# GenomicBreeding/GenomicBreedingModels.jl

Hardware: AMD Instinct MI355X
Metric: GRM+GBLUP genotype-cells/s (n x p) (higher is better)
Workload: dtype f64

## Files before the change

### genomicbreedingmodels.jl_amd/csrc/chol.hip

```cpp
#include <cstdlib>
#include <string>

#include "chol_device.h"

namespace gbm {

constexpr int NB = kCholNB;
constexpr int MAXRHS = 63;

int launch_chol_update(double* G, int64_t ldg, int64_t k0, int64_t nb, int64_t gdim, double* Ld, double* Dinv,
                       int32_t* info, int64_t next_k0, int rank, int nranks, hipStream_t s, int64_t col_lo = 0,
                       int64_t col_hi = INT64_MAX, int64_t row_lo = 0, int64_t row_hi = INT64_MAX);
int launch_chol_row_update(double* G, int64_t ldg, int64_t k0, int kch, int64_t gdim, double* Ld, double* Dinv,
                           int32_t* info, hipStream_t s, ColKeep keep = ColKeep{});
int64_t chol_small_lim();
void chol_refresh_tuning();
int64_t chol_flow_flag_bytes(int64_t gdim);
bool chol_flow_enabled(int64_t npad);
int launch_chol_flow(double* G, int64_t ldg, int64_t gdim, double* Ld, double* Dinv, void* flag_block, int32_t* info,
                     hipStream_t s);

__global__ void __launch_bounds__(256) prepare_v_kernel(double* __restrict__ G, int64_t ld, int64_t n,
                                                        int64_t npad, int64_t gdim, double inv_q,
                                                        const int64_t* __restrict__ q_dev, double lambda,
                                                        const double* __restrict__ Y, int64_t ldy, int64_t nrhs,
                                                        int32_t* __restrict__ info, ColKeep keep) {
  const int64_t i = blockIdx.x;
  if (i == 0 && threadIdx.x == 0) *info = 0;
  if (q_dev) inv_q = 1.0 / (double)(*q_dev);
  double* row = G + i * ld;
  const int64_t jbeg = (i / NB) * NB;
  for (int64_t j = jbeg + threadIdx.x; j < gdim; j += 256) {
    if (keep.nranks > 1 && !col_kept(keep, j)) continue;
    double v = 0.0;
    if (i < npad) {
      if (j < i) v = 0.0;
      else if (j < npad) v = (i < n && j < n) ? row[j] * inv_q + (i == j ? lambda : 0.0) : (i == j ? 1.0 : 0.0);
      else if (i < n) {
        const int64_t t = j - npad;
        v = t == 0 ? 1.0 : (t <= nrhs ? Y[(t - 1) * ldy + i] : 0.0);
      }
    }
    row[j] = v;
  }
}

// ... 664 lines not shown
    const char* e = ::gbm::knob(name);
    return e ? (int64_t)atoll(e) : dflt;
  };
  const int64_t g4 = lim("GBM_CHOL_G4_LIM", 8192), g8 = lim("GBM_CHOL_G8_LIM", 8192),
                g16 = lim("GBM_CHOL_G16_LIM", 16384);
  const int64_t k0 = kb * NB;
  if (g16 >= 0 && kb + 16 < nb && gdim - (k0 + 16 * NB) > g16) return 16;
  if (g8 >= 0 && kb + 8 < nb && gdim - (k0 + 8 * NB) > g8) return 8;
  if (g4 >= 0 && kb + 4 < nb && gdim - (k0 + 4 * NB) > g4) return 4;
  if (kb + 2 < nb && gdim - (k0 + 2 * NB) > chol_small_lim()) return 2;
  return 1;
}

int solve_prepare(double* G, int64_t ldg, int64_t n, double inv_q, const int64_t* q_dev, double lambda,
                  const double* Y, int64_t ldy, int64_t nrhs, int32_t* info, void* workspace, hipStream_t s,
                  bool factor_first = true, ColKeep keep = ColKeep{}) {
  const int64_t npad = npad_of(n), gdim = gdim_of(n);
  const SolveWs w = solve_ws(workspace, npad);
  chol_refresh_tuning();
  prepare_v_kernel<<<(unsigned)gdim, 256, 0, s>>>(G, ldg, n, npad, gdim, inv_q, q_dev, lambda, Y, ldy, nrhs, info,
                                                  keep);
  GBM_LAUNCH_CHECK();
  if (!factor_first) return GBM_OK;
  factor_diag_kernel<<<1, 256, 0, s>>>(G, ldg, 0, w.Ld, w.Dinv, info);
  GBM_LAUNCH_CHECK();
  return GBM_OK;
}

static bool group_kernel_enabled() {
  const char* e = ::gbm::knob("GBM_CHOL_GROUP_KERNEL");
  return !e || atoi(e) != 0;
}

int solve_group_panels(double* G, int64_t ldg, int64_t n, int64_t kb, ColKeep keep, int32_t* info, void* workspace,
                       hipStream_t s, int64_t* g_out) {
  const int64_t npad = npad_of(n), gdim = gdim_of(n), nb = npad / NB;
// ... 120 lines not shown
    GBM_TRY(solve_prepare(G, ldg, n, inv_q, q_dev, lambda, Y, ldy, nrhs, info, workspace, s, false));
    const SolveWs w = solve_ws(workspace, npad);
    GBM_TRY(launch_chol_flow(G, ldg, gdim_of(n), w.Ld, w.Dinv, w.flow, info, s));
    return solve_finish(G, ldg, n, Y, ldy, nrhs, lambda, A_out, gebv, lda, mu, info, workspace, s);
  }
  GBM_TRY(solve_prepare(G, ldg, n, inv_q, q_dev, lambda, Y, ldy, nrhs, info, workspace, s));
  const int64_t nb = npad / NB;
  for (int64_t kb = 0; kb < nb;) {
    int64_t g = 1;
    GBM_TRY(solve_group(G, ldg, n, kb, info, workspace, s, &g));
    kb += g;
  }
  return solve_finish(G, ldg, n, Y, ldy, nrhs, lambda, A_out, gebv, lda, mu, info, workspace, s);
}

extern "C" int gbm_dev_chol_prepare(double* G, int64_t ldg, int64_t n, double inv_q, const int64_t* q_dev,
                                    double lambda, const double* Y, int64_t ldy, int64_t nrhs, int32_t* info,
                                    void* workspace, int64_t ws_bytes, void* stream) {
  if (!Y || ldy < n || nrhs < 1 || nrhs > MAXRHS || !(lambda > 0.0) || !(q_dev || inv_q > 0.0))
    return fail(GBM_E_ARG, "gbm_dev_chol_prepare: bad arguments");
  GBM_TRY(check_solve_args(G, ldg, n, info, workspace, ws_bytes, "gbm_dev_chol_prepare"));
  return solve_prepare(G, ldg, n, inv_q, q_dev, lambda, Y, ldy, nrhs, info, workspace, (hipStream_t)stream);
}

extern "C" int gbm_dev_chol_prepare_cols(double* G, int64_t ldg, int64_t n, double inv_q, const int64_t* q_dev,
                                         double lambda, const double* Y, int64_t ldy, int64_t nrhs, int rank,
                                         int nranks, int32_t* info, void* workspace, int64_t ws_bytes, void* stream) {
  if (!Y || ldy < n || nrhs < 1 || nrhs > MAXRHS || !(lambda > 0.0) || !(q_dev || inv_q > 0.0) || nranks < 1 ||
      rank < 0 || rank >= nranks)
    return fail(GBM_E_ARG, "gbm_dev_chol_prepare_cols: bad arguments");
// ... 191 lines not shown
```

### genomicbreedingmodels.jl_amd/csrc/chol_device.h

```cpp
#pragma once
#include "gbm_internal.h"

namespace gbm {

typedef double d4 __attribute__((ext_vector_type(4)));

constexpr int CNB = 64;
constexpr int PS = CNB + 16;

struct ColKeep {
  int32_t rank = 0, nranks = 1;
  int64_t keep_hi = 0, rhs0 = INT64_MAX;
};
__device__ __forceinline__ bool col_kept(const ColKeep& k, int64_t col) {
  return k.nranks == 1 || col < k.keep_hi || col >= k.rhs0 || (col / 128) % k.nranks == k.rank;
}

__device__ __forceinline__ double rsqrt_nr(double a) {
  double y = __builtin_amdgcn_rsq(a);
  const double h = 0.5 * a * y;
  return y * fma(-h, y, 1.5);
}
__device__ __forceinline__ double rcp_nr(double a) {
  double y = __builtin_amdgcn_rcp(a);
  const double e = fma(-a, y, 1.0);
  return fma(y, e, y);
}
__device__ __forceinline__ double readlane_d(double x, int lane) {
  union {
    double d;
// ... 188 lines not shown
```

### genomicbreedingmodels.jl_amd/csrc/chol_flow.hip

```cpp
#include <atomic>
#include <cstdlib>
#include <map>
#include <mutex>
#include <type_traits>
#include <vector>

#include "chol_device.h"

namespace gbm {

namespace {

typedef double dbl2 __attribute__((ext_vector_type(2)));
typedef unsigned int u4 __attribute__((ext_vector_type(4)));
typedef unsigned int u2 __attribute__((ext_vector_type(2)));
constexpr int FT = 64;
constexpr int32_t kPairBit = 0x8000;
constexpr int kTraceRec = 32;
constexpr int kSc1 = 16;

__device__ __forceinline__ __amdgpu_buffer_rsrc_t rsrc(const void* p, int64_t bytes) {
  return __builtin_amdgcn_make_buffer_rsrc(const_cast<void*>(p), (short)0, (int)bytes, 0x00020000);
}
__device__ __forceinline__ dbl2 ld2(__amdgpu_buffer_rsrc_t r, uint32_t voff, uint32_t soff) {
  return __builtin_bit_cast(dbl2, __builtin_amdgcn_raw_buffer_load_b128(r, (int)voff, (int)soff, kSc1));
}
__device__ __forceinline__ double ld1(__amdgpu_buffer_rsrc_t r, uint32_t voff) {
  return __builtin_bit_cast(double, __builtin_amdgcn_raw_buffer_load_b64(r, (int)voff, 0, kSc1));
}
__device__ __forceinline__ void st2(__amdgpu_buffer_rsrc_t r, uint32_t voff, dbl2 v) {
  __builtin_amdgcn_raw_buffer_store_b128(__builtin_bit_cast(u4, v), r, (int)voff, 0, kSc1);
}
__device__ __forceinline__ void st1(__amdgpu_buffer_rsrc_t r, uint32_t voff, double v) {
  __builtin_amdgcn_raw_buffer_store_b64(__builtin_bit_cast(u2, v), r, (int)voff, 0, kSc1);
}

#ifndef GBM_FLOW_POST_EVERY
#define GBM_FLOW_POST_EVERY 4
#endif
#ifndef GBM_FLOW_STAGES
#define GBM_FLOW_STAGES 8
#endif
#ifndef GBM_FLOW_POLL_SLEEP
#define GBM_FLOW_POLL_SLEEP 4
#endif


constexpr int32_t kPartial = 1, kAssisted = 2, kFinal = 3;
__device__ __forceinline__ bool flag_at_least(const int32_t* f, int32_t v) {
// ... 287 lines not shown
  asm volatile("s_waitcnt vmcnt(0)" ::: "memory");
  if (lane == 0) __hip_atomic_fetch_or(leaf_bits, 1 << w, __ATOMIC_RELAXED, __HIP_MEMORY_SCOPE_AGENT);
  after_own(w);
  lds_sync();
  const double dg = X[lane * PS + lane];
  const unsigned long long bm = __ballot(!(dg > 0.0) || !isfinite(dg));
  return bm ? (int)__builtin_ctzll(bm) : -1;
}


template <bool kTrace>
__global__ void __launch_bounds__(256, 1)
chol_flow_kernel(double* __restrict__ G, int64_t ld, int nbc, double* __restrict__ Ld, double* __restrict__ Dinv,
                 int32_t* __restrict__ queue, int32_t* __restrict__ flags, int32_t* __restrict__ info,
                 const int32_t* __restrict__ order, int nwork, int xn_defer, int64_t* __restrict__ trace,
                 int trace_roles) {
  __shared__ __attribute__((aligned(16))) double X[FT * PS];
  __shared__ __attribute__((aligned(16))) double X2[FT * PS];
  __shared__ __attribute__((aligned(16))) double X3[FT * PS];
  __shared__ __attribute__((aligned(16))) double Dl[4 * 256];
  __shared__ ChainSync sy;
  __shared__ int s_task;
  const int tid = threadIdx.x, lane = tid & 63, wave = tid >> 6;
  const int wr = wave >> 1, wc = wave & 1;
  const int fr = lane >> 4, fc = lane & 15;
  const int nb = nbc - 1;
  const int ntasks = nbc * (nbc + 1) / 2;
  const int64_t gbytes_rowblk = (int64_t)FT * ld * 8;
  const __amdgpu_buffer_rsrc_t rLd = rsrc(Ld, (int64_t)nb * FT * CNB * 8);
  const __amdgpu_buffer_rsrc_t rDi = rsrc(Dinv, (int64_t)nb * FT * 16 * 8);

  auto store_lower = [&](const double* Xs, int64_t i0, int64_t j0) {
    const int row = tid & 63, quarter = tid >> 6;
    double* dl = G + (j0 + row) * ld + i0 + quarter * 16;
#pragma unroll
    for (int e = 0; e < 16; e += 2) {
      dbl2 v;
      v.x = Xs[(quarter * 16 + e) * PS + row];
      v.y = Xs[(quarter * 16 + e + 1) * PS + row];
      *reinterpret_cast<dbl2*>(dl + e) = v;
    }
  };

  if (blockIdx.x == 0) {
    if (tid == 0) {
      sy.rows = sy.b12 = sy.b13 = sy.pro = sy.x2 = sy.dl = 0;
    }
    for (int e = tid; e < FT * FT / 2; e += 256) {
      const int r = e >> 5, c2 = (e & 31) * 2;
      *reinterpret_cast<dbl2*>(&X[r * PS + c2]) = *reinterpret_cast<const dbl2*>(G + (int64_t)r * ld + c2);
    }
    lds_sync();
    double* Xa = X;
    double* Xn = X3;
    for (int i = 0; i < nb; i++) {
      const int64_t i0 = (int64_t)i * FT, j0 = i0 + FT;
      const bool next_diag = i + 1 < nb;
      int64_t* const crec = kTrace && (trace_roles & 1) ? trace + (int64_t)(ntasks + i) * kTraceRec : nullptr;
      auto cstamp = [&](int e, int64_t v) {
        if (kTrace && crec && tid == 0) crec[3 + e] = v;
      };
      cstamp(0, (int64_t)__builtin_amdgcn_s_memrealtime());
      __builtin_amdgcn_s_setprio(2);
      auto fetch_tile = [&](double* dst, int64_t r0, const int32_t* f, int32_t ready, auto&& gate) {
        const __amdgpu_buffer_rsrc_t rG = rsrc(G + r0 * ld, gbytes_rowblk);
// ... 181 lines not shown
  auto worker_task = [&](auto nt, int t, int i, int j) {
    constexpr int NT = decltype(nt)::value;
    const bool diag = i == j;
    const bool nbr = j == i + 1;
    if ((diag && i < nb) || nbr || j == i + 2) __builtin_amdgcn_s_setprio(2);
    const int64_t i0 = (int64_t)i * FT, j0 = (int64_t)j * FT;
    const int kend = ((diag && i < nb) || (nbr && i >= 1)) ? i - 1 : i;
    int64_t* const wrec = kTrace && (trace_roles & 4) ? trace + (int64_t)t * kTraceRec : nullptr;
    auto wstamp = [&](int e) {
      if (kTrace && wrec && tid == 0) wrec[3 + e] = (int64_t)__builtin_amdgcn_s_memrealtime();
    };
    wstamp(0);

    d4 acc[NT][2][2];
#pragma unroll
    for (int q = 0; q < NT; q++)
#pragma unroll
      for (int m = 0; m < 2; m++)
#pragma unroll
        for (int r = 0; r < 4; r++) {
          const int64_t row = i0 + 32 * wr + 2 * (fr + 4 * r) + m;
          const dbl2 v = *reinterpret_cast<const dbl2*>(G + row * ld + j0 + q * FT + 32 * wc + 2 * fc);
          acc[q][m][0][r] = v.x;
          acc[q][m][1][r] = v.y;
        }

    constexpr int GS = NT == 1 ? 32 : 21;
    constexpr unsigned long long GM = (1ull << GS) - 1;
    int kr = 0;
    bool gave_up = false;
    auto ready_upto = [&](int k) {
      for (int64_t it = 0; k >= kr && !gave_up; it++) {
        const int g = lane / GS, kk = kr + lane % GS;
        int ok = 1;
        if (g <= NT && kk < kend) ok = flag_at_least(flags + (int64_t)kk * nbc + (g == 0 ? i : j + g - 1), kFinal) ? 1 : 0;
        const unsigned long long bm = __ballot(ok);
        unsigned long long all = bm & GM;
#pragma unroll
        for (int q = 1; q <= NT; q++) all &= (bm >> (q * GS)) & GM;
        kr += all == GM ? GS : __builtin_ctzll(~all);
// ... 300 lines not shown

}

int64_t chol_flow_flag_bytes(int64_t gdim) {
  const int64_t nbc = gdim / FT;
  return round_up(16 + nbc * nbc * 4, 16);
}

bool chol_flow_enabled(int64_t npad) {
  const char* e = ::gbm::knob("GBM_CHOL_FLOW_MAX");
  const int64_t lim = e ? (int64_t)atoll(e) : (int64_t)12288;
  return npad <= lim;
}

int launch_chol_flow(double* G, int64_t ldg, int64_t gdim, double* Ld, double* Dinv, void* flag_block, int32_t* info,
                     hipStream_t s) {
  const int64_t nbc = gdim / FT;
  const int64_t ntasks = nbc * (nbc + 1) / 2;
  if (nbc < 2 || (int64_t)FT * ldg * 8 > 0x7fffffff || nbc * nbc > 0x3fffffff || nbc > 0x7fff)
    return fail(GBM_E_ARG, "dataflow Cholesky: matrix too large for 32-bit buffer offsets");
  const int32_t* order = nullptr;
  int nwork = 0;
  GBM_TRY(flow_order_dev((int)nbc, &order, &nwork));
  GBM_HIP_TRY(hipMemsetAsync(flag_block, 0, (size_t)chol_flow_flag_bytes(gdim), s));
  if (::gbm::knob("GBM_TEST_CHOL_FLOW_ABORT")) GBM_HIP_TRY(hipMemsetAsync(info, 0xFF, sizeof(int32_t), s));
  const char* ew = ::gbm::knob("GBM_CHOL_FLOW_WGS");
  const int64_t workers = ew && atoll(ew) > 0 ? atoll(ew) : flow_cus() - 2;
  const unsigned grid = (unsigned)(2 + (nwork < workers ? nwork : (workers < 1 ? 1 : workers)));
  int32_t* q = (int32_t*)flag_block;
  const char* ex = ::gbm::knob("GBM_CHOL_FLOW_XN");
  const int xn_defer = ex && atoi(ex) == 0 ? 0 : 1;
  if (::gbm::knob("GBM_CHOL_FLOW_TRACE")) {
    const int64_t nrec = ntasks + nbc;
    if (g_trace_cap < nrec) {
      if (g_trace) (void)hipFree(g_trace);
      g_trace = nullptr;
      GBM_HIP_TRY(hipMalloc((void**)&g_trace, (size_t)nrec * kTraceRec * 8));
      g_trace_cap = nrec;
    }
    GBM_HIP_TRY(hipMemsetAsync(g_trace, 0, (size_t)nrec * kTraceRec * 8, s));
    g_trace_n = nrec;
    const int tm = atoi(::gbm::knob("GBM_CHOL_FLOW_TRACE"));
    const int roles = tm > 1 ? (tm & 7) : 7;
    if (::gbm::knob("GBM_CHOL_FLOW_TRACE_PLAIN"))
      chol_flow_kernel<false><<<grid, 256, 0, s>>>(G, ldg, (int)nbc, Ld, Dinv, q, q + 4, info, order, nwork, xn_defer, nullptr, 0);
    else
    chol_flow_kernel<true><<<grid, 256, 0, s>>>(G, ldg, (int)nbc, Ld, Dinv, q, q + 4, info, order, nwork, xn_defer, g_trace, roles);
  } else {
    chol_flow_kernel<false><<<grid, 256, 0, s>>>(G, ldg, (int)nbc, Ld, Dinv, q, q + 4, info, order, nwork, xn_defer, nullptr, 0);
  }
  GBM_LAUNCH_CHECK();
  return GBM_OK;
}

}

extern "C" int64_t gbm_debug_chol_flow_trace(int64_t* host, int64_t cap) {
  using namespace gbm;
  if (!g_trace || !host) return 0;
  const int64_t n = g_trace_n < cap ? g_trace_n : cap;
  if (hipDeviceSynchronize() != hipSuccess || hipMemcpy(host, g_trace, (size_t)n * kTraceRec * 8, hipMemcpyDeviceToHost) != hipSuccess)
    return -1;
  return n;
}
// ... 18 lines not shown
```

### genomicbreedingmodels.jl_amd/csrc/gbm_internal.h

```cpp
#pragma once
#include <hip/hip_runtime.h>
#include <stdint.h>
#include <functional>
#include <string>
#include <vector>

#include "../../include/gbm.h"

namespace gbm {

constexpr int64_t kNPadTile = 128;
constexpr int64_t kRhsRows = 64;
constexpr int kCholNB = 64;

inline int64_t round_up(int64_t x, int64_t m) { return (x + m - 1) / m * m; }
inline int64_t npad_of(int64_t n) { return round_up(n < 1 ? 1 : n, kNPadTile); }
inline int64_t gdim_of(int64_t n) { return npad_of(n) + kRhsRows; }

void set_error(const std::string& msg);
int fail(int code, const std::string& msg);
const std::string& last_error();

const char* knob(const char* name);
int64_t knob_i64(const char* name, int64_t def);
// ... 5 lines not shown
      return ::gbm::fail(GBM_E_HIP, std::string("HIP error '") + hipGetErrorString(e_) +       \
                                        "' at " __FILE__ ":" + std::to_string(__LINE__) + " (" #expr ")"); \
  } while (0)

#define GBM_LAUNCH_CHECK() GBM_HIP_TRY(hipGetLastError())

#define GBM_TRY(expr)              \
  do {                             \
    int rc_ = (expr);              \
    if (rc_ != GBM_OK) return rc_; \
  } while (0)

int launch_grm(const double* Zt, int64_t ldz, int64_t p, int64_t n, double* G, int64_t ldg,
               void* ws, int64_t ws_bytes, hipStream_t s, int accum = 0, int32_t* err_out = nullptr);
bool grm_can_accumulate(int64_t n, int64_t p);
int launch_standardize_rows(const double* Xt, int64_t ldx, int64_t p, int64_t n, double* Zt, int64_t ldz, double* mean,
                            double* sd, int32_t* keep, int64_t* q_dev, hipStream_t s, bool beside_tiles = false);
bool standardize_fits_beside_tiles(int64_t n);
int64_t grm_workspace_bytes(int64_t n, int64_t p);
int launch_grm_export(const double* G, int64_t ldg, int64_t n, double inv_q, double* out, int64_t ldo, hipStream_t s);
int launch_predict(const double* Xt, int64_t ldx, int64_t p, int64_t n, const double* b, int64_t ldb, int64_t nrhs,
                   double* partial, int64_t nchunks, double* out, int64_t ldo, hipStream_t s);
int64_t predict_chunks(int64_t n, int64_t p);
int launch_add_inplace(double* a, const double* b, int64_t n, hipStream_t s);
int launch_standardize_i8(const int8_t* D, int64_t ldd, int64_t p, int64_t n, int ploidy, double* Zt, int64_t ldz,
                          double* mean, double* sd, int32_t* keep, int64_t* q_dev, hipStream_t s);
int launch_marker_rows(const double* Zt, int64_t ldz, int64_t p, int64_t n, const double* A, int64_t lda, int64_t nrhs,
                       double inv_q, const int64_t* q_dev, const double* sd, const int32_t* keep, double* B,
                       int64_t ldb, hipStream_t s);
int launch_marker_rows_i8(const int8_t* D, int64_t ldd, int64_t p, int64_t n, int ploidy, const double* A, int64_t lda,
// ... 101 lines not shown
```

### genomicbreedingmodels.jl_amd/csrc/grm.hip

```cpp
#include <algorithm>
#include <atomic>
#include <cmath>
#include <cstdio>
#include <cstdlib>
#include <map>
#include <mutex>
#include <queue>
#include <tuple>
#include <vector>

#include "chol_device.h"

namespace gbm {

constexpr int BT = 128;
constexpr int BK = 16;
constexpr int WPS = 2;
constexpr int LROW = BT + 2;
constexpr int STAGE = 2 * BK * LROW;

__device__ __forceinline__ void tile_of(int64_t t, int64_t& ti, int64_t& tj) {
  int64_t r = (int64_t)((sqrt(8.0 * (double)t + 1.0) - 1.0) * 0.5);
  while ((r + 1) * (r + 2) / 2 <= t) r++;
  while (r * (r + 1) / 2 > t) r--;
// ... 1079 lines not shown
    return GBM_OK;
  }
  if (g.sb.carry) {
    int32_t err = 0;
    GBM_HIP_TRY(hipMemcpyAsync(&err, (const int32_t*)ws + g.ntiles, sizeof(int32_t), hipMemcpyDeviceToHost, s));
    GBM_HIP_TRY(hipStreamSynchronize(s));
    if (err < 0)
      return fail(GBM_E_HIP, "GRM in-order carry accumulation: an inter-workgroup wait timed out (G is invalid)");
    return GBM_OK;
  }
  grm_slab_reduce_kernel<<<(unsigned)g.ntiles, 256, 0, s>>>((const double*)ws, g.ntiles, g.sb.n, G, ldg, accum);
  GBM_LAUNCH_CHECK();
  return GBM_OK;
}

int launch_grm(const double* Zt, int64_t ldz, int64_t p, int64_t n, double* G, int64_t ldg, void* ws,
               int64_t ws_bytes, hipStream_t s, int accum, int32_t* err_out) {
  if (accum && !grm_can_accumulate(n, p)) return fail(GBM_E_ARG, "GRM: accumulation needs the slab split");
  int rc = launch_grm_syrk(Zt, ldz, p, n, G, ldg, ws, ws_bytes, s, accum);
  if (rc != GBM_OK) return rc;
  return launch_grm_reduce(n, p, G, ldg, ws, s, accum, err_out);
}

bool grm_can_accumulate(int64_t n, int64_t p) {
  const GrmPlan g = plan(n, p);
  return g.sb.n > 1;
}

}

// ... 113 lines not shown
```

### genomicbreedingmodels.jl_amd/gbm/_lib.py

```python
from __future__ import annotations

import ctypes
import os
import threading

import numpy as np

ABI_VERSION = 212
GBM_OK = 0
GBM_E_ARG = -1
GBM_E_NOTPD = -2
GBM_E_HIP = -3
GBM_E_RCCL = -4
GBM_E_OOM = -5
GBM_E_NODEV = -6
GBM_E_DATA = -7

LIB_PATH = os.environ.get("GBM_LIBGBM") or os.path.join(os.path.dirname(os.path.abspath(__file__)), "libgbm.so")

EXPORTS = (
    "gbm_version", "gbm_last_error", "gbm_device_count", "gbm_device_allocations", "gbm_release_device_cache",
    "gbm_gblup_fit", "gbm_gblup_fit_reml", "gbm_gblup_fit_dosage_i8", "gbm_gblup_fit_synthetic", "gbm_grm", "gbm_grm_ploidy_aware", "gbm_colstats", "gbm_predict",
    "gbm_dev_npad", "gbm_dev_gdim", "gbm_dev_grm_workspace", "gbm_dev_solve_workspace",
    "gbm_dev_synth_genotypes", "gbm_dev_expand_dosage_i8", "gbm_dev_standardize", "gbm_dev_grm",
# ... 6 lines not shown
    "gbm_dev_chol_prepare", "gbm_dev_chol_prepare_cols", "gbm_dev_chol_group_size", "gbm_dev_chol_group", "gbm_dev_chol_factor_diag",
    "gbm_dev_chol_strip_doubles", "gbm_dev_chol_strip_pack", "gbm_dev_chol_strip_unpack", "gbm_dev_chol_finish",
    "gbm_dev_grm_packed_size", "gbm_dev_grm_pack", "gbm_dev_grm_unpack",
    "gbm_debug_brr_stats", "gbm_debug_brr_shape", "gbm_debug_brr_trace", "gbm_debug_chol_flow_trace",
    "gbm_dev_synth_dosage_i8", "gbm_dev_standardize_i8", "gbm_dev_grm_accumulate", "gbm_dev_marker_effects_i8",
    "gbm_debug_oom_retries", "gbm_dev_chol_group_panels", "gbm_dev_chol_group_update", "gbm_dev_chol_strip_unpack_rows", "gbm_dev_chol_lower_copy",
    "gbm_dev_chol_area_doubles", "gbm_dev_chol_area_pack", "gbm_dev_chol_area_unpack",
    "gbm_dev_chol_group_update_cols", "gbm_dev_chol_group_update_tiles", "gbm_dev_grm_exact_workspace", "gbm_dev_grm_exact_i8",
    "gbm_gblup_fit_ex", "gbm_gblup_fit_reml_ex", "gbm_gblup_fit_dosage_i8_ex", "gbm_gblup_fit_synthetic_ex",
    "gbm_session_set_grm_mode", "gbm_session_grm_used", "gbm_debug_rccl_calls", "gbm_debug_xg_choose", "gbm_debug_chol_flow_order",
    "gbm_debug_chol_flow_order_check", "gbm_debug_chol_flow_order_size", "gbm_dev_grm_exact_status", "gbm_debug_set",
    "gbm_dev_whiten_rows", "gbm_session_gwas", "gbm_session_enet_path", "gbm_dev_standardize_grm_syrk",
    "gbm_dev_grm_symmetrize", "gbm_dev_rows_times_sym", "gbm_dev_rows_times_sym_workspace", "gbm_session_pcs",
    "gbm_debug_sym_eig", "gbm_session_pair_scan", "gbm_bayes_fit_ordinal", "gbm_debug_ordinal_math",
    "gbm_bayes_fit_multi", "gbm_debug_bayes_multi_stats", "gbm_bayes_fit_multi_rows", "gbm_debug_bayes_rows_stats",
)

GBM_GRM_DEFAULT, GBM_GRM_FP64, GBM_GRM_EXACT, GBM_GRM_AUTO, GBM_GRM_DROPIN = -1, 0, 1, 2, 3
GBM_PCS_GRM, GBM_PCS_REFERENCE = 0, 1
PCS_KINDS = {"grm": GBM_PCS_GRM, "reference": GBM_PCS_REFERENCE}
PAIR_OPS = {"mult": 0, "addnorm": 1, "raise": 2, "square": 3, "invoneplus": 4, "log10epsdivlog10eps": 5}
GRM_MODES = {None: GBM_GRM_DEFAULT, "default": GBM_GRM_DEFAULT, "fp64": GBM_GRM_FP64, "exact": GBM_GRM_EXACT,
             "auto": GBM_GRM_AUTO, "dropin": GBM_GRM_DROPIN}


def grm_mode(mode) -> int:
    if isinstance(mode, int) and mode in GRM_MODES.values():
        return mode
    try:
        return GRM_MODES[mode]
# ... 102 lines not shown
    lib.gbm_dev_grm_exact_workspace.argtypes = [I64, I64]
    lib.gbm_dev_grm_exact_i8.restype = I32
    lib.gbm_dev_grm_exact_i8.argtypes = [P, I64, I64, I64, I32, P, I64, P, P, P, P, I32, P, I64, P, P]
    lib.gbm_dev_marker_effects_i8.argtypes = [P, I64, I64, I64, I32, P, I64, I64, D, P, P, P, P, P, I64, P, P]
    for f in ("gbm_dev_grm", "gbm_dev_grm_syrk", "gbm_dev_grm_accumulate"):
        getattr(lib, f).restype = I32
        getattr(lib, f).argtypes = [P, I64, I64, I64, P, I64, P, I64, P]
    lib.gbm_dev_standardize_grm_syrk.restype = I32
    lib.gbm_dev_standardize_grm_syrk.argtypes = [P, I64, I64, I64, P, I64, P, P, P, P, P, I64, P, I64, P]
    lib.gbm_dev_grm_reduce.restype = I32
    lib.gbm_dev_grm_reduce.argtypes = [I64, I64, P, I64, P, P]
    lib.gbm_dev_grm_slices.restype = I32
    lib.gbm_dev_grm_slices.argtypes = [I64, I64]
    lib.gbm_dev_gblup_solve.restype = I32
    lib.gbm_dev_gblup_solve.argtypes = [P, I64, I64, D, P, D, P, I64, I64, P, P, I64, P, P, P, I64, P]
    lib.gbm_dev_marker_effects.restype = I32
    lib.gbm_dev_marker_effects.argtypes = [P, I64, I64, I64, P, I64, I64, D, P, P, P, P, P, I64, P, P]
    lib.gbm_dev_standardize_gather.restype = I32
    lib.gbm_dev_standardize_gather.argtypes = [P, I64, I64, P, I64, P, I64, P, P, P, P, I32, P]
    lib.gbm_dev_gblup_terms.restype = I32
    lib.gbm_dev_gblup_terms.argtypes = [P, I64, I64, I64, P, P, P]
    lib.gbm_session_create.restype = I32
    lib.gbm_session_create.argtypes = [P, I64, I64, I64, I32, ctypes.POINTER(P)]
    lib.gbm_session_create_synthetic.restype = I32
    lib.gbm_session_create_synthetic.argtypes = [U64, I64, I64, I32, ctypes.POINTER(P)]
    lib.gbm_session_create_dosage_i8.restype = I32
    lib.gbm_session_create_dosage_i8.argtypes = [P, I64, I64, I64, I32, I32, ctypes.POINTER(P)]
    lib.gbm_session_destroy.restype = None
    lib.gbm_session_destroy.argtypes = [P]
    lib.gbm_session_gblup_fit.restype = I32
# ... 149 lines not shown
```

### genomicbreedingmodels.jl_amd/gbm/sharded.py

```python
from __future__ import annotations

import ctypes

import numpy as np

from . import _lib


class TorchComm:

    def __init__(self, force: bool = False):
        import torch.distributed as dist
        self.dist = dist
        self.world_size = dist.get_world_size() if dist.is_initialized() else 1
        self.rank = dist.get_rank() if dist.is_initialized() else 0
        self.force = bool(force) and dist.is_initialized()

    def all_reduce_sum(self, t):
        if self.world_size > 1 or self.force:
            self.dist.all_reduce(t, op=self.dist.ReduceOp.SUM)

    def all_gather(self, t):
        import torch
        out = torch.empty(self.world_size * t.numel(), dtype=t.dtype, device=t.device)
# ... 197 lines not shown

def _written_by_standardize(name):
    attr = "_" + name

    def get(self):
        if self._std_pending:
            self._standardize_now()
        return getattr(self, attr)

    def put(self, value):
        setattr(self, attr, value)

    return property(get, put)


class HipShardStages:

    def __init__(self, n: int, p_local: int, nrhs: int = 1, lambda_: float = 1.0, device: int = 0):
        import torch
        self.torch = torch
        self.lib = _lib.load()
        self.n, self.p, self.nrhs, self.lam = n, p_local, nrhs, float(lambda_)
        self.dev = torch.device("cuda", device)
        lib = self.lib
        self.npad = lib.gbm_dev_npad(n)
        self.gdim = lib.gbm_dev_gdim(n)
        f64 = dict(dtype=torch.float64, device=self.dev)
        self._alloc_rows(f64)
        self.mean = torch.empty(p_local, **f64)
        self.sd = torch.empty(p_local, **f64)
# ... 55 lines not shown
    sd = _written_by_standardize("sd")
    keep = _written_by_standardize("keep")
    q = _written_by_standardize("q")

    def standardize(self):
        self._q.zero_()
        self._std_pending = True

    def _standardize_now(self):
        self._std_pending = False
        _lib.check(self.lib.gbm_dev_standardize(self._p(self.X), self.npad, self.p, self.n, self._p(self._Z), self.npad,
                                                self._p(self._mean), self._p(self._sd), self._p(self._keep),
                                                self._p(self._q), self._stream()), "standardize")

    def grm_syrk(self):
        if self._std_pending:
            self._std_pending = False
            _lib.check(self.lib.gbm_dev_standardize_grm_syrk(
                self._p(self.X), self.npad, self.p, self.n, self._p(self._Z), self.npad, self._p(self._mean),
                self._p(self._sd), self._p(self._keep), self._p(self._q), self._p(self.G), self.gdim,
                self._p(self.ws_grm), self.ws_grm_bytes, self._stream()), "standardize_grm_syrk")
            return
        _lib.check(self.lib.gbm_dev_grm_syrk(self._p(self.Z), self.npad, self.p, self.n, self._p(self.G), self.gdim,
                                             self._p(self.ws_grm), self.ws_grm_bytes, self._stream()), "grm_syrk")

    def grm_reduce(self):
        _lib.check(self.lib.gbm_dev_grm_reduce(self.n, self.p, self._p(self.G), self.gdim, self._p(self.ws_grm),
                                               self._stream()), "grm_reduce")

    def grm_rows(self):
        return self.G[: self.npad]

    def grm_pack(self):
        if getattr(self, "Gp", None) is None:
            self.Gp = self.torch.empty(self.lib.gbm_dev_grm_packed_size(self.n) + 1, dtype=self.torch.float64,
                                       device=self.dev)
        _lib.check(self.lib.gbm_dev_grm_pack(self._p(self.G), self.gdim, self.n, self._p(self.Gp), self._stream()),
                   "grm_pack")
        self.Gp[-1:].copy_(self.q)
        return self.Gp

    def grm_unpack(self):
        _lib.check(self.lib.gbm_dev_grm_unpack(self._p(self.Gp), self.n, self._p(self.G), self.gdim, self._stream()),
                   "grm_unpack")
        self.q.copy_(self.Gp[-1:])

    def solve(self):
        _lib.check(self.lib.gbm_dev_gblup_solve(self._p(self.G), self.gdim, self.n, 0.0, self._p(self.q), self.lam,
                                                self._p(self.Y), self.npad, self.nrhs, self._p(self.A),
                                                self._p(self.gebv), self.npad, self._p(self.mu), self._p(self.info),
                                                self._p(self.ws_solve), self.ws_solve_bytes, self._stream()), "solve")

    def chol_prepare(self):
        _lib.check(self.lib.gbm_dev_chol_prepare(self._p(self.G), self.gdim, self.n, 0.0, self._p(self.q), self.lam,
                                                 self._p(self.Y), self.npad, self.nrhs, self._p(self.info),
                                                 self._p(self.ws_solve), self.ws_solve_bytes, self._stream()),
                   "chol_prepare")

    def chol_prepare_cols(self, rank: int, nranks: int):
        _lib.check(self.lib.gbm_dev_chol_prepare_cols(self._p(self.G), self.gdim, self.n, 0.0, self._p(self.q),
                                                      self.lam, self._p(self.Y), self.npad, self.nrhs, rank, nranks,
                                                      self._p(self.info), self._p(self.ws_solve), self.ws_solve_bytes,
# ... 227 lines not shown
```

### include/gbm.h

```cpp
#ifndef GBM_H
#define GBM_H

#include <stdint.h>

#ifdef __cplusplus
extern "C" {
#endif

#define GBM_VERSION 212

#define GBM_OK 0
#define GBM_E_ARG (-1)
#define GBM_E_NOTPD (-2)
#define GBM_E_HIP (-3)
#define GBM_E_RCCL (-4)
#define GBM_E_OOM (-5)
#define GBM_E_NODEV (-6)
#define GBM_E_DATA (-7)

#define GBM_GRM_DEFAULT (-1)
#define GBM_GRM_FP64 0
#define GBM_GRM_EXACT 1
#define GBM_GRM_AUTO 2
#define GBM_GRM_DROPIN 3
// ... 93 lines not shown
int gbm_dev_grm_syrk(const double* Zt, int64_t ldz, int64_t p, int64_t n, double* G, int64_t ldg,
                     void* workspace, int64_t ws_bytes, void* stream);
int gbm_dev_grm_reduce(int64_t n, int64_t p, double* G, int64_t ldg, const void* workspace, void* stream);
int gbm_dev_standardize_grm_syrk(const double* Xt, int64_t ldx, int64_t p, int64_t n, double* Zt, int64_t ldz,
                                 double* mean, double* sd, int32_t* keep, int64_t* q_dev, double* G, int64_t ldg,
                                 void* workspace, int64_t ws_bytes, void* stream);
int64_t gbm_dev_grm_packed_size(int64_t n);
int gbm_dev_grm_pack(const double* G, int64_t ldg, int64_t n, double* packed, void* stream);
int gbm_dev_grm_unpack(const double* packed, int64_t n, double* G, int64_t ldg, void* stream);
int gbm_dev_grm_slices(int64_t n, int64_t p);

int gbm_dev_gblup_solve(double* G, int64_t ldg, int64_t n, double inv_q, const int64_t* q_dev, double lambda,
                        const double* Y, int64_t ldy, int64_t nrhs,
                        double* A_out, double* gebv, int64_t lda, double* mu, int32_t* info,
                        void* workspace, int64_t ws_bytes, void* stream);

int gbm_dev_chol_prepare(double* G, int64_t ldg, int64_t n, double inv_q, const int64_t* q_dev, double lambda,
                         const double* Y, int64_t ldy, int64_t nrhs, int32_t* info, void* workspace,
                         int64_t ws_bytes, void* stream);
int gbm_dev_chol_prepare_cols(double* G, int64_t ldg, int64_t n, double inv_q, const int64_t* q_dev, double lambda,
                              const double* Y, int64_t ldy, int64_t nrhs, int rank, int nranks, int32_t* info,
                              void* workspace, int64_t ws_bytes, void* stream);
int64_t gbm_dev_chol_group_size(int64_t n, int64_t kb);
int gbm_dev_chol_group(double* G, int64_t ldg, int64_t n, int64_t kb, int rank, int nranks, int32_t* info,
                       void* workspace, int64_t ws_bytes, void* stream);
int gbm_dev_chol_group_panels(double* G, int64_t ldg, int64_t n, int64_t kb, int rank, int nranks, int32_t* info,
                              void* workspace, int64_t ws_bytes, void* stream);
int gbm_dev_chol_group_update(double* G, int64_t ldg, int64_t n, int64_t kb, int rank, int nranks, int32_t* info,
                              void* workspace, int64_t ws_bytes, void* stream);
int gbm_dev_chol_group_update_cols(double* G, int64_t ldg, int64_t n, int64_t kb, int rank, int nranks,
// ... 169 lines not shown
```

Before: 12.12 billion.

## Fuse GRM slab reduction into dataflow Cholesky tile loads

Defers the GRM split-K slab reduction. The dataflow Cholesky kernel now sums the per-slice slabs itself when it first loads each tile left of the edge column, and applies the scale and lambda shift at that point, rather than reading a G that a separate reduce kernel had already written. This removes one full pass that writes G and reads it back, and it shrinks the prepare kernel to the columns past c0. In exchange, each tile load inside the critical factorization path now performs several strided nontemporal reads, which may lengthen the per-task latency. It also adds lazy-reduce state in the Python wrapper so G is still reduced when something reads it directly.

```diff
diff --git a/genomicbreedingmodels.jl_amd/csrc/chol.hip b/genomicbreedingmodels.jl_amd/csrc/chol.hip
--- a/genomicbreedingmodels.jl_amd/csrc/chol.hip
+++ b/genomicbreedingmodels.jl_amd/csrc/chol.hip
@@ -18,18 +18,19 @@
 int64_t chol_flow_flag_bytes(int64_t gdim);
 bool chol_flow_enabled(int64_t npad);
 int launch_chol_flow(double* G, int64_t ldg, int64_t gdim, double* Ld, double* Dinv, void* flag_block, int32_t* info,
-                     hipStream_t s);
+                     hipStream_t s, const VSource& vs = VSource{});
 
 __global__ void __launch_bounds__(256) prepare_v_kernel(double* __restrict__ G, int64_t ld, int64_t n,
                                                         int64_t npad, int64_t gdim, double inv_q,
                                                         const int64_t* __restrict__ q_dev, double lambda,
                                                         const double* __restrict__ Y, int64_t ldy, int64_t nrhs,
-                                                        int32_t* __restrict__ info, ColKeep keep) {
+                                                        int32_t* __restrict__ info, ColKeep keep, int64_t c0) {
   const int64_t i = blockIdx.x;
   if (i == 0 && threadIdx.x == 0) *info = 0;
   if (q_dev) inv_q = 1.0 / (double)(*q_dev);
   double* row = G + i * ld;
-  const int64_t jbeg = (i / NB) * NB;
+  const int64_t jdiag = (i / NB) * NB;
+  const int64_t jbeg = jdiag > c0 ? jdiag : c0;
   for (int64_t j = jbeg + threadIdx.x; j < gdim; j += 256) {
     if (keep.nranks > 1 && !col_kept(keep, j)) continue;
     double v = 0.0;
@@ -724,12 +725,12 @@
 
 int solve_prepare(double* G, int64_t ldg, int64_t n, double inv_q, const int64_t* q_dev, double lambda,
                   const double* Y, int64_t ldy, int64_t nrhs, int32_t* info, void* workspace, hipStream_t s,
-                  bool factor_first = true, ColKeep keep = ColKeep{}) {
+                  bool factor_first = true, ColKeep keep = ColKeep{}, int64_t c0 = 0) {
   const int64_t npad = npad_of(n), gdim = gdim_of(n);
   const SolveWs w = solve_ws(workspace, npad);
   chol_refresh_tuning();
   prepare_v_kernel<<<(unsigned)gdim, 256, 0, s>>>(G, ldg, n, npad, gdim, inv_q, q_dev, lambda, Y, ldy, nrhs, info,
-                                                  keep);
+                                                  keep, c0);
   GBM_LAUNCH_CHECK();
   if (!factor_first) return GBM_OK;
   factor_diag_kernel<<<1, 256, 0, s>>>(G, ldg, 0, w.Ld, w.Dinv, info);
@@ -880,6 +881,45 @@
   return solve_finish(G, ldg, n, Y, ldy, nrhs, lambda, A_out, gebv, lda, mu, info, workspace, s);
 }
 
+extern "C" int gbm_dev_gblup_solve_slabs(double* G, int64_t ldg, int64_t n, int64_t p, const void* ws_grm,
+                                         int64_t ws_grm_bytes, double inv_q, const int64_t* q_dev, double lambda,
+                                         const double* Y, int64_t ldy, int64_t nrhs, double* A_out, double* gebv,
+                                         int64_t lda, double* mu, int32_t* info, void* workspace, int64_t ws_bytes,
+                                         void* stream) {
+  const int64_t npad = npad_of(n);
+  hipStream_t s = (hipStream_t)stream;
+  if (p < 1 || n < 1 || !G || ldg < npad)
+    return fail(GBM_E_ARG, "gbm_dev_gblup_solve_slabs: bad arguments (need p >= 1 and the G of gbm_dev_grm_syrk)");
+  const GrmSlabSource src = grm_slab_source(n, p);
+  const bool slabs = src.usable && chol_flow_enabled(npad) && knob_i64("GBM_SOLVE_SLABS", 1) != 0;
+  if (!slabs) {
+    GBM_TRY(launch_grm_reduce(n, p, G, ldg, ws_grm, s, 0, nullptr));
+    return gbm_dev_gblup_solve(G, ldg, n, inv_q, q_dev, lambda, Y, ldy, nrhs, A_out, gebv, lda, mu, info, workspace,
+                               ws_bytes, stream);
+  }
+  if (!Y || !A_out || !gebv || !mu || ldy < n || lda < npad || nrhs < 1 || nrhs > MAXRHS || !(lambda > 0.0) ||
+      !(q_dev || inv_q > 0.0))
+    return fail(GBM_E_ARG, "gbm_dev_gblup_solve_slabs: bad arguments (need ldg >= gdim(n), lda >= npad(n), "
+                           "1 <= nrhs <= 63, lambda > 0, inv_q > 0)");
+  GBM_TRY(check_solve_args(G, ldg, n, info, workspace, ws_bytes, "gbm_dev_gblup_solve_slabs"));
+  if (!ws_grm || ((uintptr_t)ws_grm & 15) || ws_grm_bytes < grm_workspace_bytes(n, p))
+    return fail(GBM_E_ARG, "gbm_dev_gblup_solve_slabs: the GRM workspace of gbm_dev_grm_syrk is required");
+  GBM_TRY(launch_grm_edge_reduce_pending(n, p, G, ldg, ws_grm, s));
+  GBM_TRY(solve_prepare(G, ldg, n, inv_q, q_dev, lambda, Y, ldy, nrhs, info, workspace, s, false, ColKeep{}, src.c0));
+  VSource vs;
+  vs.slab = (const double*)ws_grm + src.slab_off;
+  vs.ntiles = src.ntiles;
+  vs.nslices = src.nslices;
+  vs.c0_tile64 = (int32_t)(src.c0 / NB);
+  vs.n = n;
+  vs.q_dev = q_dev;
+  vs.inv_q = inv_q;
+  vs.lambda = lambda;
+  const SolveWs w = solve_ws(workspace, npad);
+  GBM_TRY(launch_chol_flow(G, ldg, gdim_of(n), w.Ld, w.Dinv, w.flow, info, s, vs));
+  return solve_finish(G, ldg, n, Y, ldy, nrhs, lambda, A_out, gebv, lda, mu, info, workspace, s);
+}
+
 extern "C" int gbm_dev_chol_prepare(double* G, int64_t ldg, int64_t n, double inv_q, const int64_t* q_dev,
                                     double lambda, const double* Y, int64_t ldy, int64_t nrhs, int32_t* info,
                                     void* workspace, int64_t ws_bytes, void* stream) {
diff --git a/genomicbreedingmodels.jl_amd/csrc/chol_device.h b/genomicbreedingmodels.jl_amd/csrc/chol_device.h
--- a/genomicbreedingmodels.jl_amd/csrc/chol_device.h
+++ b/genomicbreedingmodels.jl_amd/csrc/chol_device.h
@@ -14,6 +14,21 @@
 };
 __device__ __forceinline__ bool col_kept(const ColKeep& k, int64_t col) {
   return k.nranks == 1 || col < k.keep_hi || col >= k.rhs0 || (col / 128) % k.nranks == k.rank;
+}
+
+struct VSource {
+  const double* slab = nullptr;
+  int64_t ntiles = 0;
+  int32_t nslices = 0, c0_tile64 = 0;
+  int64_t n = 0;
+  const int64_t* q_dev = nullptr;
+  double inv_q = 0.0, lambda = 0.0;
+};
+__device__ __forceinline__ double v_entry(double g, int64_t i, int64_t j, int64_t n, double inv_q, double lambda) {
+  double v = 0.0;
+  if (j < i) v = 0.0;
+  else v = (i < n && j < n) ? g * inv_q + (i == j ? lambda : 0.0) : (i == j ? 1.0 : 0.0);
+  return v;
 }
 
 __device__ __forceinline__ double rsqrt_nr(double a) {
diff --git a/genomicbreedingmodels.jl_amd/csrc/chol_flow.hip b/genomicbreedingmodels.jl_amd/csrc/chol_flow.hip
--- a/genomicbreedingmodels.jl_amd/csrc/chol_flow.hip
+++ b/genomicbreedingmodels.jl_amd/csrc/chol_flow.hip
@@ -33,6 +33,57 @@
 }
 __device__ __forceinline__ void st1(__amdgpu_buffer_rsrc_t r, uint32_t voff, double v) {
   __builtin_amdgcn_raw_buffer_store_b64(__builtin_bit_cast(u2, v), r, (int)voff, 0, kSc1);
+}
+
+#ifndef GBM_FLOW_SLAB_RANGES
+#define GBM_FLOW_SLAB_RANGES 3
+#endif
+constexpr int kSlabT = 128;
+template <int CNT>
+__device__ __forceinline__ void slab_ranges_add(const char* p, int64_t stride, const uint32_t (&off)[8], dbl2 (&acc)[8]) {
+  dbl2 v[CNT][8];
+#pragma unroll
+  for (int u = 0; u < CNT; u++)
+#pragma unroll
+    for (int e = 0; e < 8; e++)
+      v[u][e] = __builtin_nontemporal_load(reinterpret_cast<const dbl2*>(p + u * stride + off[e]));
+  __builtin_amdgcn_sched_barrier(0);
+#pragma unroll
+  for (int u = 0; u < CNT; u++)
+#pragma unroll
+    for (int e = 0; e < 8; e++) {
+      acc[e].x += v[u][e].x;
+      acc[e].y += v[u][e].y;
+    }
+}
+__device__ __forceinline__ void v_tile_from_slabs(const VSource& vs, double inv_q, int i, int j, const int (&row)[8],
+                                                  const int (&col)[8], dbl2 (&out)[8]) {
+  constexpr int64_t per = (int64_t)kSlabT * kSlabT;
+  const int64_t t = (int64_t)(j >> 1) * ((j >> 1) + 1) / 2 + (i >> 1);
+  const char* p = reinterpret_cast<const char*>(vs.slab + t * per + (i & 1) * (FT * kSlabT) + (j & 1) * FT);
+  const int64_t stride = vs.ntiles * per * 8;
+  uint32_t off[8];
+  dbl2 acc[8];
+#pragma unroll
+  for (int e = 0; e < 8; e++) {
+    off[e] = (uint32_t)(row[e] * kSlabT + col[e]) * 8u;
+    acc[e] = (dbl2){0.0, 0.0};
+  }
+  constexpr int RG = GBM_FLOW_SLAB_RANGES;
+  static_assert(RG >= 1 && RG <= 4, "ranges in flight");
+  int s = 0;
+  for (; s + RG <= vs.nslices; s += RG) slab_ranges_add<RG>(p + s * stride, stride, off, acc);
+  const int rem = vs.nslices - s;
+  if (RG > 3 && rem == 3) slab_ranges_add<3>(p + s * stride, stride, off, acc);
+  else if (RG > 2 && rem == 2) slab_ranges_add<2>(p + s * stride, stride, off, acc);
+  else if (RG > 2 && rem == 1) slab_ranges_add<1>(p + s * stride, stride, off, acc);
+  else if (RG == 2 && rem == 1) slab_ranges_add<1>(p + s * stride, stride, off, acc);
+  const int64_t i0 = (int64_t)i * FT, j0 = (int64_t)j * FT;
+#pragma unroll
+  for (int e = 0; e < 8; e++) {
+    out[e].x = v_entry(acc[e].x, i0 + row[e], j0 + col[e], vs.n, inv_q, vs.lambda);
+    out[e].y = v_entry(acc[e].y, i0 + row[e], j0 + col[e] + 1, vs.n, inv_q, vs.lambda);
+  }
 }
 
 #ifndef GBM_FLOW_POST_EVERY
@@ -350,7 +401,7 @@
 chol_flow_kernel(double* __restrict__ G, int64_t ld, int nbc, double* __restrict__ Ld, double* __restrict__ Dinv,
                  int32_t* __restrict__ queue, int32_t* __restrict__ flags, int32_t* __restrict__ info,
                  const int32_t* __restrict__ order, int nwork, int xn_defer, int64_t* __restrict__ trace,
-                 int trace_roles) {
+                 int trace_roles, VSource vs) {
   __shared__ __attribute__((aligned(16))) double X[FT * PS];
   __shared__ __attribute__((aligned(16))) double X2[FT * PS];
   __shared__ __attribute__((aligned(16))) double X3[FT * PS];
@@ -365,6 +416,13 @@
   const int64_t gbytes_rowblk = (int64_t)FT * ld * 8;
   const __amdgpu_buffer_rsrc_t rLd = rsrc(Ld, (int64_t)nb * FT * CNB * 8);
   const __amdgpu_buffer_rsrc_t rDi = rsrc(Dinv, (int64_t)nb * FT * 16 * 8);
+  double vs_inv_q = vs.inv_q;
+  if (vs.slab) {
+    if (vs.q_dev) vs_inv_q = 1.0 / (double)(*vs.q_dev);
+    const uint64_t b = __builtin_bit_cast(uint64_t, vs_inv_q);
+    const uint32_t lo = __builtin_amdgcn_readfirstlane((uint32_t)b), hi = __builtin_amdgcn_readfirstlane((uint32_t)(b >> 32));
+    vs_inv_q = __builtin_bit_cast(double, ((uint64_t)hi << 32) | lo);
+  }
 
   auto store_lower = [&](const double* Xs, int64_t i0, int64_t j0) {
     const int row = tid & 63, quarter = tid >> 6;
@@ -382,9 +440,26 @@
     if (tid == 0) {
       sy.rows = sy.b12 = sy.b13 = sy.pro = sy.x2 = sy.dl = 0;
     }
-    for (int e = tid; e < FT * FT / 2; e += 256) {
-      const int r = e >> 5, c2 = (e & 31) * 2;
-      *reinterpret_cast<dbl2*>(&X[r * PS + c2]) = *reinterpret_cast<const dbl2*>(G + (int64_t)r * ld + c2);
+    if (vs.slab && vs.c0_tile64 > 0) {
+      int row[8], col[8];
+      dbl2 v[8];
+#pragma unroll
+      for (int k = 0; k < 8; k++) {
+        const int e = tid + 256 * k;
+        row[k] = e >> 5;
+        col[k] = (e & 31) * 2;
+      }
+      v_tile_from_slabs(vs, vs_inv_q, 0, 0, row, col, v);
+#pragma unroll
+      for (int k = 0; k < 8; k++) {
+        *reinterpret_cast<dbl2*>(&X[row[k] * PS + col[k]]) = v[k];
+        *reinterpret_cast<dbl2*>(G + (int64_t)row[k] * ld + col[k]) = v[k];
+      }
+    } else {
+      for (int e = tid; e < FT * FT / 2; e += 256) {
+        const int r = e >> 5, c2 = (e & 31) * 2;
+        *reinterpret_cast<dbl2*>(&X[r * PS + c2]) = *reinterpret_cast<const dbl2*>(G + (int64_t)r * ld + c2);
+      }
     }
     lds_sync();
     double* Xa = X;
@@ -596,7 +671,29 @@
 
     d4 acc[NT][2][2];
 #pragma unroll
-    for (int q = 0; q < NT; q++)
+    for (int q = 0; q < NT; q++) {
+      if (vs.slab && j + q < vs.c0_tile64) {
+        int ol = lane;
+        asm volatile("" : "+v"(ol));
+        int row[8], col[8];
+        dbl2 v[8];
+#pragma unroll
+        for (int m = 0; m < 2; m++)
+#pragma unroll
+          for (int r = 0; r < 4; r++) {
+            row[m * 4 + r] = 32 * wr + 2 * ((ol >> 4) + 4 * r) + m;
+            col[m * 4 + r] = 32 * wc + 2 * (ol & 15);
+          }
+        v_tile_from_slabs(vs, vs_inv_q, i, j + q, row, col, v);
+#pragma unroll
+        for (int m = 0; m < 2; m++)
+#pragma unroll
+          for (int r = 0; r < 4; r++) {
+            acc[q][m][0][r] = v[m * 4 + r].x;
+            acc[q][m][1][r] = v[m * 4 + r].y;
+          }
+        continue;
+      }
 #pragma unroll
       for (int m = 0; m < 2; m++)
 #pragma unroll
@@ -606,6 +703,7 @@
           acc[q][m][0][r] = v.x;
           acc[q][m][1][r] = v.y;
         }
+    }
 
     constexpr int GS = NT == 1 ? 32 : 21;
     constexpr unsigned long long GM = (1ull << GS) - 1;
@@ -936,8 +1034,11 @@
 }
 
 int launch_chol_flow(double* G, int64_t ldg, int64_t gdim, double* Ld, double* Dinv, void* flag_block, int32_t* info,
-                     hipStream_t s) {
+                     hipStream_t s, const VSource& vs) {
   const int64_t nbc = gdim / FT;
+  if (vs.slab && (vs.nslices < 2 || vs.ntiles < 1 || vs.c0_tile64 < 0 || vs.c0_tile64 > nbc - 1 || (vs.c0_tile64 & 1) ||
+                  (int64_t)(vs.c0_tile64 / 2) * (vs.c0_tile64 / 2 + 1) / 2 > vs.ntiles || ((uintptr_t)vs.slab & 15)))
+    return fail(GBM_E_ARG, "dataflow Cholesky: bad slab source");
   const int64_t ntasks = nbc * (nbc + 1) / 2;
   if (nbc < 2 || (int64_t)FT * ldg * 8 > 0x7fffffff || nbc * nbc > 0x3fffffff || nbc > 0x7fff)
     return fail(GBM_E_ARG, "dataflow Cholesky: matrix too large for 32-bit buffer offsets");
@@ -965,11 +1066,11 @@
     const int tm = atoi(::gbm::knob("GBM_CHOL_FLOW_TRACE"));
     const int roles = tm > 1 ? (tm & 7) : 7;
     if (::gbm::knob("GBM_CHOL_FLOW_TRACE_PLAIN"))
-      chol_flow_kernel<false><<<grid, 256, 0, s>>>(G, ldg, (int)nbc, Ld, Dinv, q, q + 4, info, order, nwork, xn_defer, nullptr, 0);
+      chol_flow_kernel<false><<<grid, 256, 0, s>>>(G, ldg, (int)nbc, Ld, Dinv, q, q + 4, info, order, nwork, xn_defer, nullptr, 0, vs);
     else
-    chol_flow_kernel<true><<<grid, 256, 0, s>>>(G, ldg, (int)nbc, Ld, Dinv, q, q + 4, info, order, nwork, xn_defer, g_trace, roles);
+    chol_flow_kernel<true><<<grid, 256, 0, s>>>(G, ldg, (int)nbc, Ld, Dinv, q, q + 4, info, order, nwork, xn_defer, g_trace, roles, vs);
   } else {
-    chol_flow_kernel<false><<<grid, 256, 0, s>>>(G, ldg, (int)nbc, Ld, Dinv, q, q + 4, info, order, nwork, xn_defer, nullptr, 0);
+    chol_flow_kernel<false><<<grid, 256, 0, s>>>(G, ldg, (int)nbc, Ld, Dinv, q, q + 4, info, order, nwork, xn_defer, nullptr, 0, vs);
   }
   GBM_LAUNCH_CHECK();
   return GBM_OK;
diff --git a/genomicbreedingmodels.jl_amd/csrc/gbm_internal.h b/genomicbreedingmodels.jl_amd/csrc/gbm_internal.h
--- a/genomicbreedingmodels.jl_amd/csrc/gbm_internal.h
+++ b/genomicbreedingmodels.jl_amd/csrc/gbm_internal.h
@@ -43,6 +43,17 @@
 int launch_grm(const double* Zt, int64_t ldz, int64_t p, int64_t n, double* G, int64_t ldg,
                void* ws, int64_t ws_bytes, hipStream_t s, int accum = 0, int32_t* err_out = nullptr);
 bool grm_can_accumulate(int64_t n, int64_t p);
+int launch_grm_reduce(int64_t n, int64_t p, double* G, int64_t ldg, const void* ws, hipStream_t s, int accum,
+                      int32_t* err_out);
+struct GrmSlabSource {
+  bool usable = false;
+  int64_t slab_off = 0, ntiles = 0, c0 = 0;
+  int32_t nslices = 0;
+  bool edge_reduce_pending = false;
+  static int64_t tile_index(int64_t I, int64_t J) { return J * (J + 1) / 2 + I; }
+};
+GrmSlabSource grm_slab_source(int64_t n, int64_t p);
+int launch_grm_edge_reduce_pending(int64_t n, int64_t p, double* G, int64_t ldg, const void* ws, hipStream_t s);
 int launch_standardize_rows(const double* Xt, int64_t ldx, int64_t p, int64_t n, double* Zt, int64_t ldz, double* mean,
                             double* sd, int32_t* keep, int64_t* q_dev, hipStream_t s, bool beside_tiles = false);
 bool standardize_fits_beside_tiles(int64_t n);
diff --git a/genomicbreedingmodels.jl_amd/csrc/grm.hip b/genomicbreedingmodels.jl_amd/csrc/grm.hip
--- a/genomicbreedingmodels.jl_amd/csrc/grm.hip
+++ b/genomicbreedingmodels.jl_amd/csrc/grm.hip
@@ -1117,6 +1117,28 @@
   return GBM_OK;
 }
 
+GrmSlabSource grm_slab_source(int64_t n, int64_t p) {
+  const GrmPlan g = plan(n, p);
+  GrmSlabSource v;
+  v.usable = !g.sb.carry && !g.sb.fuse && g.sb.n >= 2;
+  v.slab_off = 0;
+  v.ntiles = g.ntiles;
+  v.nslices = g.sb.n;
+  v.c0 = g.sb.er > 0 ? g.sb.e0 : npad_of(n);
+  v.edge_reduce_pending = g.sb.er > 0 && !g.edge_concurrent;
+  return v;
+}
+
+int launch_grm_edge_reduce_pending(int64_t n, int64_t p, double* G, int64_t ldg, const void* ws, hipStream_t s) {
+  const GrmPlan g = plan(n, p);
+  if (!(g.sb.er > 0 && !g.edge_concurrent)) return GBM_OK;
+  if (!ws) return fail(GBM_E_ARG, "gbm_dev_grm_reduce: workspace required");
+  grm_edge_reduce_kernel<<<(unsigned)((n * g.sb.er + 255) / 256), 256, 0, s>>>((const double*)ws + g.sb.eslab_off, n,
+                                                                               g.sb, G, ldg, 0);
+  GBM_LAUNCH_CHECK();
+  return GBM_OK;
+}
+
 int launch_grm(const double* Zt, int64_t ldz, int64_t p, int64_t n, double* G, int64_t ldg, void* ws,
                int64_t ws_bytes, hipStream_t s, int accum, int32_t* err_out) {
   if (accum && !grm_can_accumulate(n, p)) return fail(GBM_E_ARG, "GRM: accumulation needs the slab split");
diff --git a/genomicbreedingmodels.jl_amd/gbm/_lib.py b/genomicbreedingmodels.jl_amd/gbm/_lib.py
--- a/genomicbreedingmodels.jl_amd/gbm/_lib.py
+++ b/genomicbreedingmodels.jl_amd/gbm/_lib.py
@@ -44,6 +44,7 @@
     "gbm_dev_grm_symmetrize", "gbm_dev_rows_times_sym", "gbm_dev_rows_times_sym_workspace", "gbm_session_pcs",
     "gbm_debug_sym_eig", "gbm_session_pair_scan", "gbm_bayes_fit_ordinal", "gbm_debug_ordinal_math",
     "gbm_bayes_fit_multi", "gbm_debug_bayes_multi_stats", "gbm_bayes_fit_multi_rows", "gbm_debug_bayes_rows_stats",
+    "gbm_dev_gblup_solve_slabs",
 )
 
 GBM_GRM_DEFAULT, GBM_GRM_FP64, GBM_GRM_EXACT, GBM_GRM_AUTO, GBM_GRM_DROPIN = -1, 0, 1, 2, 3
@@ -176,6 +177,8 @@
     lib.gbm_dev_grm_slices.argtypes = [I64, I64]
     lib.gbm_dev_gblup_solve.restype = I32
     lib.gbm_dev_gblup_solve.argtypes = [P, I64, I64, D, P, D, P, I64, I64, P, P, I64, P, P, P, I64, P]
+    lib.gbm_dev_gblup_solve_slabs.restype = I32
+    lib.gbm_dev_gblup_solve_slabs.argtypes = [P, I64, I64, I64, P, I64, D, P, D, P, I64, I64, P, P, I64, P, P, P, I64, P]
     lib.gbm_dev_marker_effects.restype = I32
     lib.gbm_dev_marker_effects.argtypes = [P, I64, I64, I64, P, I64, I64, D, P, P, P, P, P, I64, P, P]
     lib.gbm_dev_standardize_gather.restype = I32
diff --git a/genomicbreedingmodels.jl_amd/gbm/sharded.py b/genomicbreedingmodels.jl_amd/gbm/sharded.py
--- a/genomicbreedingmodels.jl_amd/gbm/sharded.py
+++ b/genomicbreedingmodels.jl_amd/gbm/sharded.py
@@ -235,6 +235,20 @@
     return property(get, put)
 
 
+def _written_by_grm_reduce(name):
+    attr = "_" + name
+
+    def get(self):
+        if self._reduce_pending:
+            self._grm_reduce_now()
+        return getattr(self, attr)
+
+    def put(self, value):
+        setattr(self, attr, value)
+
+    return property(get, put)
+
+
 class HipShardStages:
 
     def __init__(self, n: int, p_local: int, nrhs: int = 1, lambda_: float = 1.0, device: int = 0):
@@ -320,18 +334,26 @@
                                                 self._p(self._q), self._stream()), "standardize")
 
     def grm_syrk(self):
+        self._reduce_pending = False
         if self._std_pending:
             self._std_pending = False
             _lib.check(self.lib.gbm_dev_standardize_grm_syrk(
                 self._p(self.X), self.npad, self.p, self.n, self._p(self._Z), self.npad, self._p(self._mean),
-                self._p(self._sd), self._p(self._keep), self._p(self._q), self._p(self.G), self.gdim,
+                self._p(self._sd), self._p(self._keep), self._p(self._q), self._p(self._G), self.gdim,
                 self._p(self.ws_grm), self.ws_grm_bytes, self._stream()), "standardize_grm_syrk")
             return
-        _lib.check(self.lib.gbm_dev_grm_syrk(self._p(self.Z), self.npad, self.p, self.n, self._p(self.G), self.gdim,
+        _lib.check(self.lib.gbm_dev_grm_syrk(self._p(self.Z), self.npad, self.p, self.n, self._p(self._G), self.gdim,
                                              self._p(self.ws_grm), self.ws_grm_bytes, self._stream()), "grm_syrk")
 
+    _reduce_pending = False
+    G = _written_by_grm_reduce("G")
+
     def grm_reduce(self):
-        _lib.check(self.lib.gbm_dev_grm_reduce(self.n, self.p, self._p(self.G), self.gdim, self._p(self.ws_grm),
+        self._reduce_pending = True
+
+    def _grm_reduce_now(self):
+        self._reduce_pending = False
+        _lib.check(self.lib.gbm_dev_grm_reduce(self.n, self.p, self._p(self._G), self.gdim, self._p(self.ws_grm),
                                                self._stream()), "grm_reduce")
 
     def grm_rows(self):
@@ -352,6 +374,14 @@
         self.q.copy_(self.Gp[-1:])
 
     def solve(self):
+        if self._reduce_pending:
+            self._reduce_pending = False
+            _lib.check(self.lib.gbm_dev_gblup_solve_slabs(
+                self._p(self._G), self.gdim, self.n, self.p, self._p(self.ws_grm), self.ws_grm_bytes, 0.0,
+                self._p(self.q), self.lam, self._p(self.Y), self.npad, self.nrhs, self._p(self.A), self._p(self.gebv),
+                self.npad, self._p(self.mu), self._p(self.info), self._p(self.ws_solve), self.ws_solve_bytes,
+                self._stream()), "solve")
+            return
         _lib.check(self.lib.gbm_dev_gblup_solve(self._p(self.G), self.gdim, self.n, 0.0, self._p(self.q), self.lam,
                                                 self._p(self.Y), self.npad, self.nrhs, self._p(self.A),
                                                 self._p(self.gebv), self.npad, self._p(self.mu), self._p(self.info),
diff --git a/include/gbm.h b/include/gbm.h
--- a/include/gbm.h
+++ b/include/gbm.h
@@ -131,6 +131,10 @@
                         const double* Y, int64_t ldy, int64_t nrhs,
                         double* A_out, double* gebv, int64_t lda, double* mu, int32_t* info,
                         void* workspace, int64_t ws_bytes, void* stream);
+int gbm_dev_gblup_solve_slabs(double* G, int64_t ldg, int64_t n, int64_t p, const void* ws_grm, int64_t ws_grm_bytes,
+                              double inv_q, const int64_t* q_dev, double lambda, const double* Y, int64_t ldy,
+                              int64_t nrhs, double* A_out, double* gebv, int64_t lda, double* mu, int32_t* info,
+                              void* workspace, int64_t ws_bytes, void* stream);
 
 int gbm_dev_chol_prepare(double* G, int64_t ldg, int64_t n, double inv_q, const int64_t* q_dev, double lambda,
                          const double* Y, int64_t ldy, int64_t nrhs, int32_t* info, void* workspace,
```

Result: no change. 12.11 billion (median of 2 runs) (-0.1%).
